# huster-wgm/SRCGAN

Hardware: AMD Instinct MI355X
Metric: paired SR-CycleGAN train images/sec at x4 256->1024 (higher is better)
Workload: dtype bf16; 1 GPU; Sat2Aerx4 paired G+D step (BASELINE configs[1]): 23-block RRDB generator + 3-layer PatchGAN, 3x256x256->3x1024x1024, batch 16/GPU; per_gpu_batch=16, global_batch=16, parallelism=dp1, gradient_exchange=none (1 rank)

## Files before the change

srcgan_amd/csrc/wgrad_dense.hip:

```cpp
#include "common.h"
#include <type_traits>
#include <stdlib.h>

struct WdSeg { int g0, g1; float* grad; float* bias; int Cin; float alpha; };
struct WdP {
    const void* dy; const void* x; float* slab;
    int B, H, W, G, C, dycoff, xcoff;
    long dypix, dyplane, xpix, xplane;
    int g_base;
    int cin_lim[4];
    int nsplit, tiles_x, tiles_y, ntiles, ncit, want_bias;
    unsigned long long* trace;
};
struct WdRedP {
    const float* slab; int nsplit, ncit, COT, g_base, nseg; WdSeg seg[8]; int accumulate;
};

typedef __attribute__((address_space(3))) s16x4 lds_s16x4_;
__device__ __forceinline__ bf16x8 tr_frag2(const char* p0, const char* p1) {
    s16x4 lo = __builtin_amdgcn_ds_read_tr16_b64_v4i16((lds_s16x4_*)(p0));
    s16x4 hi = __builtin_amdgcn_ds_read_tr16_b64_v4i16((lds_s16x4_*)(p1));
    typedef __attribute__((ext_vector_type(8))) short s16x8;
    s16x8 v = {lo[0], lo[1], lo[2], lo[3], hi[0], hi[1], hi[2], hi[3]};
    return __builtin_bit_cast(bf16x8, v);
// ... 58 lines not shown
                if (pix < DPX && oy < p.H && ox < p.W && ch < p.G)
                    src = dyb + (size_t)(oy * p.W + ox) * p.dypix + wd_chan_off<T>(p.dycoff + ch, p.dyplane);
            } else {
                const int pj = pi - MT * DPP, n = pj / XPP, pix = (pj - n * XPP) * PXP + lpx;
                const int iy = pix / IWT, ix = pix - iy * IWT;
                const int gy = oy0 - 1 + iy, gx = ox0 - 1 + ix;
                const int ch = (cit * NT + n) * 32 + part * D::EPP;
                if (pix < XPX && (unsigned)gy < (unsigned)p.H && (unsigned)gx < (unsigned)p.W && ch < p.C)
                    src = xb + (size_t)(gy * p.W + gx) * p.xpix + wd_chan_off<T>(p.xcoff + ch, p.xplane);
            }
            __builtin_amdgcn_global_load_lds((wd_gptr_t)src, (wd_lptr_t)(ls + pi * 1024), 16, 0, 0);
        }
    };

    if (t_begin < t_end) issue(t_begin, 0);
    int stage = 0;
    for (int t = t_begin; t < t_end; ++t, stage ^= 1) {
        __syncthreads();
        if (t + 1 < t_end) issue(t + 1, stage ^ 1);
        const char* my_d = smem + stage * SBYTES + wm * DBYTES;
        const char* my_x = smem + stage * SBYTES + MT * DBYTES + wn * XBYTES;
        if constexpr (std::is_same<T, float>::value) {
#pragma unroll 2
            for (int kk = 0; kk < TH * TW / 2; ++kk) {
                const int pix = 2 * kk + h;
                const int py = pix / TW, px = pix % TW;
                const float a = *(const float*)(my_d + pix * PB + r * 4);
#pragma unroll
                for (int tap = 0; tap < NTAP; ++tap) {
                    const int ky = tap / 3, kx = tap % 3;
                    const float bv = *(const float*)(my_x + ((py + ky) * IWT + px + kx) * PB + r * 4);
                    acc[tap] = __builtin_amdgcn_mfma_f32_32x32x2f32(a, bv, acc[tap], 0, 0, 0);
                }
                if (do_bias) acc[NTAP] = __builtin_amdgcn_mfma_f32_32x32x2f32(a, 1.0f, acc[NTAP], 0, 0, 0);
            }
        } else {
            const int gq = lane >> 4, idx = lane & 15, qq = idx >> 2, pp = idx & 3;
            const int choff = ((gq & 1) * 16 + 4 * pp) * 2;
            const bf16x8 ones = sg_ones16<T>();
#pragma unroll 2
            for (int kk = 0; kk < TH * 2; ++kk) {
                const int py = kk >> 1, xh = (kk & 1) * 16;
                const int px0 = xh + 8 * h + qq;
                const char* ab = my_d + (py * TW + px0) * PB + choff;
                const bf16x8 a = tr_frag2(ab, ab + 4 * PB);
#pragma unroll
                for (int tap = 0; tap < NTAP; ++tap) {
                    const int ky = tap / 3, kx = tap % 3;
                    const char* bb = my_x + ((py + ky) * IWT + px0 + kx) * PB + choff;
                    acc[tap] = sg_mfma16<T>(a, tr_frag2(bb, bb + 4 * PB), acc[tap]);
                }
                if (do_bias) acc[NTAP] = sg_mfma16<T>(a, ones, acc[NTAP]);
            }
        }
    }

    constexpr int COT = 32 * MT, CIT = 32 * NT;
    float* sp = p.slab + ((size_t)split * p.ncit + cit) * (NTAP + 1) * COT * CIT;
#pragma unroll
    for (int tap = 0; tap <= NTAP; ++tap) {
        if (tap == NTAP && !do_bias) continue;
#pragma unroll
        for (int i = 0; i < 16; ++i) {
            const int row = wm * 32 + 8 * (i >> 2) + 4 * h + (i & 3);
            sp[((size_t)tap * COT + row) * CIT + wn * 32 + r] = acc[tap][i];
        }
    }
}

typedef int wd_v4i __attribute__((ext_vector_type(4)));
__device__ __forceinline__ void wd_dma16(const void* base, int voff, int soff, wd_lptr_t lds) {
    const unsigned long long a = (unsigned long long)base;
    wd_v4i rs;
    rs[0] = __builtin_amdgcn_readfirstlane((int)(a & 0xffffffffu));
    rs[1] = __builtin_amdgcn_readfirstlane((int)((a >> 32) & 0xffffu));
    rs[2] = 0x7fffffff;
    rs[3] = 0x00020000;
    const unsigned dst = __builtin_amdgcn_readfirstlane((unsigned)(unsigned long long)lds);
    unsigned keep;
    asm volatile("s_mov_b32 %0, m0\n\ts_mov_b32 m0, %3\n\ts_nop 0\n\tbuffer_load_dwordx4 %1, %2, %4 offen lds\n\ts_mov_b32 m0, %0"
                 : "=&s"(keep) : "v"(voff), "s"(rs), "s"(dst), "s"(soff) : "memory");
}

#ifndef SG_WD_EXP
#define SG_WD_EXP 0
#endif
template <typename T, int MT, int NT, int TH>
__global__ __launch_bounds__(MT * NT * 64) void wgrad_dense_fast_k(const WdP p) {
    using D = DT<T>;
    constexpr int NW = MT * NT, TW = 32, NTAP = 9;
    constexpr int IHT = TH + 2, IWT = TW + 2;
    constexpr int PB = 64, PXP = 16;
    constexpr int DPX = TH * TW, XPX = IHT * IWT;
    constexpr int DPP = (DPX + PXP - 1) / PXP, XPP = (XPX + PXP - 1) / PXP;
    constexpr int DBYTES = DPP * 1024, XBYTES = XPP * 1024;
    constexpr int NPIECE = MT * DPP + NT * XPP, SBYTES = MT * DBYTES + NT * XBYTES;
    constexpr int IPW = (NPIECE + NW - 1) / NW;
    constexpr int OOB = 0x7fffffff;
#ifndef SG_WD_PPK
#define SG_WD_PPK 0
#endif
    constexpr int PPK = SG_WD_PPK ? SG_WD_PPK : 4;
    static_assert(IPW <= 16, "piece classes are packed 4 bits each into two registers");
    extern __shared__ __attribute__((aligned(1024))) char smem[];

    const int tid = threadIdx.x, lane = tid & 63, r = lane & 31, h = lane >> 5;
    const int wave = __builtin_amdgcn_readfirstlane(tid >> 6);
    const int wm = wave / NT, wn = wave % NT;
    int cit, split;
    {
        const int L = blockIdx.x + gridDim.x * blockIdx.y, nwg = gridDim.x * gridDim.y;
        const int xcd = L & 7, j = L >> 3;
        const int full = (nwg >> 3) * 8;
        const int per = nwg >> 3;
        const int pos = L < full ? xcd * per + j : L;
        cit = pos % p.ncit; split = pos / p.ncit;
        if (split >= p.nsplit) return;
    }
    const bool do_bias = wn == 0 && cit == 0 && p.want_bias;
#ifdef SG_WD_NO_SKIP
    const bool useful = true;
#else
    const bool useful = (cit * NT + wn) * 32 < p.cin_lim[wm] || do_bias;
#endif

#ifndef SG_WD_S16
#define SG_WD_S16 1
#endif
    constexpr bool S16 = SG_WD_S16 != 0;
    int voff[IPW]; long soff[IPW];
    unsigned cls[2] = {0u, 0u};
    {
        const int part = lane & 3, lpx = lane >> 2;
#pragma unroll
        for (int it = 0; it < IPW; ++it) {
            const int pi = it * NW + wave;
            int v = OOB; long so = 0;
            if (pi < MT * DPP) {
                const int m = pi / DPP, pix = (pi - m * DPP) * PXP + lpx;
                const int psw = S16 ? part ^ ((((pix % TW) >> 3) & 1) << 1) : part;
                const int ch = p.g_base + m * 32 + psw * D::EPP;
                if (pix < DPX && ch < p.G) v = ((pix / TW) * p.W + pix % TW) * (int)p.dypix + psw * 16;
                so = (long)wd_chan_off<T>(p.dycoff + p.g_base + m * 32, p.dyplane);
            } else if (pi < NPIECE) {
                const int pj = pi - MT * DPP, n = pj / XPP, pix = (pj - n * XPP) * PXP + lpx;
                const int iy = pix / IWT, ix = pix - iy * IWT;
                const int psw = S16 ? part ^ (((ix >> 3) & 1) << 1) : part;
                const int ch = (cit * NT + n) * 32 + psw * D::EPP;
                if (pix < XPX && ch < p.C) v = (iy * p.W + ix) * (int)p.xpix + psw * 16;
                so = (long)wd_chan_off<T>(p.xcoff + (cit * NT + n) * 32, p.xplane);
                cls[it / 8] |= (unsigned)((iy == 0) | ((iy == IHT - 1) << 1) | ((ix == 0) << 2) | ((ix == IWT - 1) << 3)) << (4 * (it % 8));
            }
            voff[it] = v;
            soff[it] = ((long)__builtin_amdgcn_readfirstlane((int)(so >> 32)) << 32) | (unsigned)__builtin_amdgcn_readfirstlane((int)(so & 0xffffffff));
        }
    }

    f32x16 acc[S16 ? 1 : NTAP + 1];
    f32x4 acq[S16 ? NTAP + 1 : 1][2][2];
#pragma unroll
    for (int a = 0; a < (S16 ? 1 : NTAP + 1); ++a)
#pragma unroll
        for (int i = 0; i < 16; ++i) acc[a][i] = 0.f;
#pragma unroll
    for (int a = 0; a < (S16 ? NTAP + 1 : 1); ++a)
#pragma unroll
        for (int i = 0; i < 16; ++i) acq[a][(i >> 3) & 1][(i >> 2) & 1][i & 3] = 0.f;

    const int t_begin = (int)((long)p.ntiles * split / p.nsplit);
    const int t_end = (int)((long)p.ntiles * (split + 1) / p.nsplit);
    int ty = t_begin % p.tiles_y, tx = (t_begin / p.tiles_y) % p.tiles_x, tb = t_begin / (p.tiles_x * p.tiles_y);
    tx = __builtin_amdgcn_readfirstlane(tx); ty = __builtin_amdgcn_readfirstlane(ty); tb = __builtin_amdgcn_readfirstlane(tb);
    const char* dyo = nullptr; const char* xo = nullptr; unsigned clm[2] = {0u, 0u};
    auto origin = [&]() {
        const long px = ((long)tb * p.H + ty * TH) * p.W + tx * TW;
        dyo = (const char*)p.dy + px * p.dypix;
        xo = (const char*)p.x + (px - p.W - 1) * p.xpix;
        const unsigned m = (unsigned)((ty == 0) | ((ty == p.tiles_y - 1) << 1) | ((tx == 0) << 2) | ((tx == p.tiles_x - 1) << 3));
        clm[0] = cls[0] & (m * 0x11111111u); clm[1] = cls[1] & (m * 0x11111111u);
    };
    auto advance = [&]() { if (++ty == p.tiles_y) { ty = 0; if (++tx == p.tiles_x) { tx = 0; ++tb; } } };
    auto piece = [&](int it, int stage) __attribute__((always_inline)) {
        const int pi = it * NW + wave;
        if (IPW * NW != NPIECE && pi >= NPIECE) return;
        int v = ((clm[it / 8] >> (4 * (it % 8))) & 15u) ? OOB : voff[it];
        if (SG_WD_EXP & 8) v = OOB;
        wd_dma16((pi < MT * DPP ? dyo : xo) + soff[it], v, 0, (wd_lptr_t)(smem + stage * SBYTES + pi * 1024));
    };

    if (t_begin < t_end) {
        origin();
#pragma unroll
        for (int it = 0; it < IPW; ++it) piece(it, 0);
    }
    const int gq = lane >> 4, idx = lane & 15, qq = idx >> 2, pp = idx & 3;
    const int choff = ((gq & 1) * 16 + 4 * pp) * 2;
    const bf16x8 ones = sg_ones16<T>();
    int stage = 0;
    for (int t = t_begin; t < t_end; ++t, stage ^= 1) {
#ifdef SG_TRACE
        const unsigned long long t_arr = __builtin_amdgcn_s_memrealtime();
        __builtin_amdgcn_s_waitcnt(0x0f70);
        const unsigned long long t_land = __builtin_amdgcn_s_memrealtime();
#endif
        __builtin_amdgcn_s_waitcnt(0x0f70);
        __syncthreads();
#ifdef SG_TRACE
        if (p.trace && blockIdx.x == 1 && blockIdx.y == 3 && lane == 0 && t - t_begin >= 8 && t - t_begin < 12)
            p.trace[160 + (t - t_begin - 8) * 8 + wave] = t_arr;
        if (p.trace && blockIdx.x == 1 && blockIdx.y == 3 && wave == 0 && lane == 0 && t - t_begin < 40) {
            p.trace[(t - t_begin) * 4 + 0] = t_arr; p.trace[(t - t_begin) * 4 + 1] = t_land; p.trace[(t - t_begin) * 4 + 2] = __builtin_amdgcn_s_memrealtime();
            p.trace[(t - t_begin) * 4 + 3] = __builtin_readcyclecounter();
        }
#endif
        const bool more = t + 1 < t_end;
        if (more) { advance(); origin(); }
        if (!useful) {
            if (more && !(SG_WD_EXP & 1)) {
#pragma unroll
                for (int it = 0; it < IPW; ++it) piece(it, stage ^ 1);
            }
            continue;
        }
        const char* my_d = smem + stage * SBYTES + wm * DBYTES;
        const char* my_x = smem + stage * SBYTES + MT * DBYTES + wn * XBYTES;
#ifndef SG_WD_PD
#define SG_WD_PD 4
#endif
        if constexpr (S16) {
            constexpr int NG = IHT * 3, PDG = 1;
            bf16x8 fa[TH][2], fb[PDG + 1][2];
            const int kq = lane >> 4;
            const int lb = (8 * kq + qq) * PB + (kq & 1) * 32 + 8 * pp;
            const int mk1 = qq + 1 >= 4 ? 32 : 0, mk2 = qq + 2 >= 4 ? 32 : 0;
            auto rd_b = [&](int G) {
                const int i2 = G / 3, kx = G % 3;
                const char* bb = my_x + (i2 * IWT + kx) * PB;
                const int l0 = lb, l1 = lb ^ (kx == 0 ? 0 : kx == 1 ? mk1 : mk2);
                fb[G % (PDG + 1)][0] = tr_frag2(bb + l0, bb + 4 * PB + l1);
                fb[G % (PDG + 1)][1] = tr_frag2(bb + (l0 ^ 32), bb + 4 * PB + (l1 ^ 32));
            };
            auto rd_a = [&](int py) {
                const char* ab = my_d + py * TW * PB;
                fa[py][0] = tr_frag2(ab + lb, ab + 4 * PB + lb);
                fa[py][1] = tr_frag2(ab + (lb ^ 32), ab + 4 * PB + (lb ^ 32));
            };
            rd_a(0); rd_b(0);
#pragma unroll
            for (int G = 0; G < NG; ++G) {
                const int i2 = G / 3, kx = G % 3;
                if (kx == 1 && i2 + 1 < TH) rd_a(i2 + 1);
                if (G + PDG < NG) rd_b(G + PDG);
                if (more) {
#pragma unroll
                    for (int j = 0; j < 2 * PPK; ++j)
                        if (2 * PPK * G + j < IPW) piece(2 * PPK * G + j, stage ^ 1);
                }
                __builtin_amdgcn_sched_barrier(0);
#pragma unroll
                for (int py = 0; py < TH; ++py) {
                    const int ky = i2 - py;
                    if (ky < 0 || ky > 2) continue;
#pragma unroll
                    for (int mb = 0; mb < 2; ++mb)
#pragma unroll
                        for (int nb = 0; nb < 2; ++nb)
                            acq[ky * 3 + kx][mb][nb] = sg_mfma16s<T>(fa[py][mb], fb[G % (PDG + 1)][nb], acq[ky * 3 + kx][mb][nb]);
                }
                if (do_bias && kx == 0 && (i2 == 0 || i2 >= IHT - 2))
#pragma unroll
                    for (int py = (i2 == 0 ? 0 : i2 == IHT - 2 ? 1 : TH / 2); py < (i2 == 0 ? 1 : i2 == IHT - 2 ? TH / 2 : TH); ++py)
#pragma unroll
                        for (int mb = 0; mb < 2; ++mb) acq[NTAP][mb][0] = sg_mfma16s<T>(fa[py][mb], ones, acq[NTAP][mb][0]);
                __builtin_amdgcn_sched_barrier(0);
            }
        } else {
        constexpr int NGRP = IHT * 3 * 2, PD = SG_WD_PD;
        bf16x8 fa[TH][2], fb[PD + 1];
        auto read_b = [&](int G) {
            const int i2 = G / 6, kx = (G % 6) / 2, xh = G % 2;
            const char* bb = my_x + (i2 * IWT + xh * 16 + 8 * h + qq + kx) * PB + choff;
            fb[G % (PD + 1)] = tr_frag2(bb, bb + 4 * PB);
        };
        auto read_a = [&](int py, int xh) {
            const char* ab = my_d + (py * TW + xh * 16 + 8 * h + qq) * PB + choff;
            fa[py][xh] = tr_frag2(ab, ab + 4 * PB);
        };
        read_a(0, 0); read_b(0); read_a(0, 1);
#pragma unroll
        for (int G = 1; G < PD; ++G) read_b(G);
        constexpr int FA_LEAD = 4;
#ifndef SG_WD_PRIO_K
#define SG_WD_PRIO_K 0
#endif
#pragma unroll
        for (int G = 0; G < NGRP; ++G) {
            if (SG_WD_PRIO_K > 0 && wave >= NW / 2) {
                if (G == 0) __builtin_amdgcn_s_setprio(1);
                if (G == SG_WD_PRIO_K) __builtin_amdgcn_s_setprio(0);
            }
            if ((G + FA_LEAD) % 6 < 2 && (G + FA_LEAD) / 6 >= 1 && (G + FA_LEAD) / 6 < TH) read_a((G + FA_LEAD) / 6, (G + FA_LEAD) % 6);
            if (G + PD < NGRP && !(SG_WD_EXP & 4)) read_b(G + PD);
            if (more && !(SG_WD_EXP & 1)) {
#pragma unroll
                for (int j = 0; j < PPK; ++j)
                    if (PPK * G + j < IPW) piece(PPK * G + j, stage ^ 1);
            }
            __builtin_amdgcn_sched_barrier(0);
#ifdef SG_TRACE
            if (G % 5 == 0 && p.trace && blockIdx.x == 1 && blockIdx.y == 3 && lane == 0 && t - t_begin == 10)
                p.trace[192 + wave * 8 + G / 5] = __builtin_amdgcn_s_memrealtime();
#endif
            const int i2 = G / 6, kx = (G % 6) / 2, xh = G % 2;
#pragma unroll
            for (int py = 0; py < TH; ++py) {
                const int ky = i2 - py;
                if (ky < 0 || ky > 2) continue;
                if (!(SG_WD_EXP & 2)) acc[ky * 3 + kx] = sg_mfma16<T>(fa[py][xh], fb[G % (PD + 1)], acc[ky * 3 + kx]);
                else asm volatile("" :: "v"(fa[py][xh]), "v"(fb[G % (PD + 1)]));
            }
            if (do_bias && kx == 0 && (i2 == 0 || i2 >= IHT - 2))
#pragma unroll
                for (int py = (i2 == 0 ? 0 : i2 == IHT - 2 ? 1 : TH / 2); py < (i2 == 0 ? 1 : i2 == IHT - 2 ? TH / 2 : TH); ++py)
                    acc[NTAP] = sg_mfma16<T>(fa[py][xh], ones, acc[NTAP]);
            __builtin_amdgcn_sched_barrier(0);
        }
        }
    }

    constexpr int COT = 32 * MT, CIT = 32 * NT;
    float* sp = p.slab + ((size_t)split * p.ncit + cit) * (NTAP + 1) * COT * CIT;
    const bool blk_needed = (cit * NT + wn) * 32 < p.cin_lim[wm];
#pragma unroll
    for (int tap = 0; tap <= NTAP; ++tap) {
        if (tap == NTAP ? !do_bias : !blk_needed) continue;
        if constexpr (S16) {
#pragma unroll
            for (int mb = 0; mb < 2; ++mb)
#pragma unroll
                for (int nb = 0; nb < 2; ++nb)
#pragma unroll
                    for (int i = 0; i < 4; ++i) {
                        const int row = wm * 32 + mb * 16 + 4 * (lane >> 4) + i;
                        sp[((size_t)tap * COT + row) * CIT + wn * 32 + nb * 16 + (lane & 15)] = acq[tap][mb][tap == NTAP ? 0 : nb][i];
                    }
        } else {
#pragma unroll
            for (int i = 0; i < 16; ++i) {
                const int row = wm * 32 + 8 * (i >> 2) + 4 * h + (i & 3);
                sp[((size_t)tap * COT + row) * CIT + wn * 32 + r] = acc[tap][i];
            }
        }
    }
}

template <int CIT>
__global__ __launch_bounds__(256) void wgrad_dense_reduce_k(const WdRedP p) {
    __shared__ float red[4][64];
    const long per_split = (long)p.ncit * 10 * p.COT * CIT;
    const int el = threadIdx.x & 63, sl = threadIdx.x >> 6;
    const long e = (long)blockIdx.x * 64 + el;
    float s = 0.f;
    bool wanted = false;
    if (e < per_split) {
        long q = e;
        const int col = (int)(q % CIT); q /= CIT;
        const int row = (int)(q % p.COT); q /= p.COT;
        const int tap = (int)(q % 10);
        const int cit = (int)(q / 10);
        const int g = p.g_base + row, ci = cit * CIT + col;
        for (int k = 0; k < p.nseg; ++k) {
            const WdSeg sg = p.seg[k];
            if (g < sg.g0 || g >= sg.g1) continue;
            wanted = tap == 9 ? (sg.bias && cit == 0 && col == 0) : (sg.grad && ci < sg.Cin);
            break;
        }
    }
    if (wanted) {
        float a0 = 0.f, a1 = 0.f, a2 = 0.f, a3 = 0.f;
        int sp = sl;
        for (; sp + 12 < p.nsplit; sp += 16) {
            a0 += p.slab[(size_t)sp * per_split + e];
            a1 += p.slab[(size_t)(sp + 4) * per_split + e];
            a2 += p.slab[(size_t)(sp + 8) * per_split + e];
            a3 += p.slab[(size_t)(sp + 12) * per_split + e];
        }
        for (; sp < p.nsplit; sp += 4) a0 += p.slab[(size_t)sp * per_split + e];
        s = (a0 + a1) + (a2 + a3);
    }
    red[sl][el] = s;
    __syncthreads();
    if (sl != 0 || !wanted) return;
    s = (red[0][el] + red[1][el]) + (red[2][el] + red[3][el]);
    long q = e;
    const int col = (int)(q % CIT); q /= CIT;
    const int row = (int)(q % p.COT); q /= p.COT;
    const int tap = (int)(q % 10);
    const int cit = (int)(q / 10);
    const int g = p.g_base + row, ci = cit * CIT + col;
    for (int k = 0; k < p.nseg; ++k) {
        const WdSeg sg = p.seg[k];
        if (g < sg.g0 || g >= sg.g1) continue;
        const int co = g - sg.g0;
        const float v = s * sg.alpha;
        if (tap == 9) {
            if (sg.bias && cit == 0 && col == 0) sg.bias[co] = p.accumulate ? sg.bias[co] + v : v;
        } else if (sg.grad && ci < sg.Cin) {
            float* gp = sg.grad + ((size_t)co * sg.Cin + ci) * 9 + tap;
            *gp = p.accumulate ? *gp + v : v;
        }
        return;
    }
}

template <typename T, int MT, int NT, int TH>
static int launch_wd(WdP p, hipStream_t st) {
    constexpr int PB = 32 * (int)sizeof(T), PXP = 64 / (PB / 16);
    constexpr size_t SMEM = 2 * 1024 * ((size_t)MT * ((TH * 32 + PXP - 1) / PXP) + (size_t)NT * (((TH + 2) * 34 + PXP - 1) / PXP));
    static_assert(SMEM <= 160 * 1024, "wgrad_dense tile exceeds LDS");
    void (*kern)(const WdP) = wgrad_dense_k<T, MT, NT, TH>;
    bool fast = false;
    if constexpr (!std::is_same<T, float>::value) {
        static const bool no_fast = sg_env("SRCGAN_WD_SLOW") != nullptr;
        const double span_dy = (double)(TH + 2) * p.W * p.dypix, span_x = (double)(TH + 4) * p.W * p.xpix;
        fast = !no_fast && p.H % TH == 0 && p.W % 32 == 0 && span_dy < 2.0e9 && span_x < 2.0e9 &&
               (p.dyplane == 64 || (p.dycoff + p.g_base) % 32 == 0) && (p.xplane == 64 || p.xcoff % 32 == 0);
        constexpr int IPWF = (MT * (TH * 2) + NT * (((TH + 2) * 34 + 15) / 16) + MT * NT - 1) / (MT * NT);
        if constexpr (IPWF <= 10) { if (fast) kern = wgrad_dense_fast_k<T, MT, NT, TH>; }
        else fast = false;
    }
    static bool attr_set[2] = {false, false};
    if (!attr_set[fast]) {
        SG_HIP(hipFuncSetAttribute((const void*)kern, hipFuncAttributeMaxDynamicSharedMemorySize, (int)SMEM));
        attr_set[fast] = true;
    }
    p.tiles_x = cdiv(p.W, 32);
    p.tiles_y = cdiv(p.H, TH);
    p.ntiles = p.B * p.tiles_x * p.tiles_y;
    if (p.nsplit > p.ntiles) p.nsplit = p.ntiles;
    char cls[96];
    snprintf(cls, sizeof(cls), "wgrad_dense<%s,MT%d,NT%d%s>", sizeof(T) == 4 ? "f32" : (__is_same(T, __bf16) ? "bf16" : "f16"), MT, NT, fast ? ",fast" : "");
    const double px = (double)p.B * p.H * p.W;
    const int rows = (p.G - p.g_base) < 32 * MT ? (p.G - p.g_base) : 32 * MT;
    double pairs = 0.0;
    for (int b = 0; b < MT; ++b) {
        const int rb = rows - 32 * b < 32 ? rows - 32 * b : 32;
        if (rb > 0) pairs += (double)rb * (p.cin_lim[b] < p.C ? p.cin_lim[b] : p.C);
    }
    const int tok = sg_prof_start(cls, 2.0 * px * 9 * pairs, px * (rows + p.C) * sizeof(T), st);
#ifdef SG_TRACE
    static unsigned long long* trace = nullptr;
    if (!trace) SG_HIP(hipMalloc(&trace, 64 * 4 * 8));
    SG_HIP(hipMemsetAsync(trace, 0, 64 * 4 * 8, st));
    p.trace = trace;
#endif
    hipLaunchKernelGGL(kern, dim3((unsigned)p.ncit, (unsigned)p.nsplit), dim3(MT * NT * 64), SMEM, st, p);
#ifdef SG_TRACE
    {
        static int dumps = 0;
        if (sg_env("SRCGAN_TRACE") && dumps < 2 && fast) {
            ++dumps;
            unsigned long long h[64 * 4];
            SG_HIP(hipStreamSynchronize(st));
            SG_HIP(hipMemcpy(h, trace, sizeof(h), hipMemcpyDeviceToHost));
            fprintf(stderr, "[trace] %s (10 ns ticks: arrive at barrier, own DMA landed, barrier exit)\n", cls);
            for (int k = 0; k < 4; ++k) {
                fprintf(stderr, "[trace] step %d arrivals by wave (rel. wave 0):", 8 + k);
                for (int w = 0; w < 8; ++w) fprintf(stderr, " %5lld", (long long)(h[160 + k * 8 + w] - h[160 + k * 8]));
                fprintf(stderr, "\n");
            }
            fprintf(stderr, "[trace] step 10: time of groups 0,5,..,35 by wave (rel. wave 0 group 0)\n");
            for (int w = 0; w < 8; ++w) {
                fprintf(stderr, "[trace]   wave %d:", w);
                for (int g = 0; g < 8; ++g) fprintf(stderr, " %5lld", (long long)(h[192 + w * 8 + g] - h[192]));
                fprintf(stderr, "\n");
            }
            for (int k = 0; k < 40 && h[k * 4]; ++k)
                fprintf(stderr, "[trace] %2d arrive %6lld landed %6lld exit %6lld  shader-clock %5.0f MHz\n", k, (long long)(h[k * 4] - h[0]), (long long)(h[k * 4 + 1] - h[0]), (long long)(h[k * 4 + 2] - h[0]),
                        k ? (double)(h[k * 4 + 3] - h[(k - 1) * 4 + 3]) / (double)(h[k * 4 + 2] - h[(k - 1) * 4 + 2]) * 100.0 : 0.0);
        }
    }
#endif
    sg_prof_stop(tok, st);
    SG_LAUNCH_CHECK();
    return p.nsplit;
}

template <typename T>
static int dispatch_wd(const WdP& p, int mt, int nt, hipStream_t st, int& nsplit_used) {
    constexpr bool F = std::is_same<T, float>::value;
    int rc = -1;
    if (nt == 4) {
        if constexpr (!F) {
            switch (mt) {
                case 1: rc = launch_wd<T, 1, 4, 4>(p, st); break;
                case 2: rc = launch_wd<T, 2, 4, 4>(p, st); break;
            }
        }
    } else if (nt == 3) {
        if constexpr (!F) {
            switch (mt) {
                case 1: rc = launch_wd<T, 1, 3, 4>(p, st); break;
                case 2: rc = launch_wd<T, 2, 3, 4>(p, st); break;
            }
        }
    } else
    switch (mt) {
        case 1: rc = launch_wd<T, 1, 2, F ? 2 : 4>(p, st); break;
        case 2: rc = launch_wd<T, 2, 2, F ? 2 : 4>(p, st); break;
        case 3: rc = launch_wd<T, 3, 2, F ? 2 : 4>(p, st); break;
        case 4: rc = launch_wd<T, 4, 2, F ? 2 : 4>(p, st); break;
    }
    if (rc < 0) SG_FAIL("srcgan_wgrad_dense: bad row-tile count %d", mt);
    nsplit_used = rc;
    return 0;
}

static int wd_nt(int mt, int cin_max, int dtype) { return (sg_is16(dtype) && mt <= 2 && cin_max > 64) ? (cin_max <= 96 ? 3 : 4) : 2; }

static int wd_nsplit(int mt, int nt, int ncit, int dtype, int B, int H, int W) {
    const int th = dtype == SRCGAN_F32 ? 2 : 4;
    const int pb = dtype == SRCGAN_F32 ? 128 : 64;
    const long lds = 2 * ((long)mt * th * 32 * pb + (long)nt * (th + 2) * 34 * pb);
    int per_cu = (int)((160 * 1024) / lds); if (per_cu < 1) per_cu = 1;
    if (per_cu * mt * nt > 16) per_cu = 16 / (mt * nt) > 0 ? 16 / (mt * nt) : 1;
    const long ntiles = (long)B * cdiv(H, th) * cdiv(W, 32);
    long cus = 256;
    if (const char* e = sg_env("SRCGAN_WD_CUS")) { const int v = atoi(e); if (v > 0 && v < 256) cus = v; }
    long ns = (cus * per_cu) / ncit;
    if (ns > ntiles) ns = ntiles;
    return (int)(ns < 1 ? 1 : ns);
}

extern "C" size_t srcgan_wgrad_dense_slab_bytes(int G, int C, int dtype, int B, int H, int W) {
    size_t mx = 0;
    for (int g_base = 0; g_base < G; g_base += 128) {
        const int rows = G - g_base < 128 ? G - g_base : 128, mt = cdiv(rows, 32);
        for (int nt = 2; nt <= (sg_is16(dtype) && mt <= 2 ? 4 : 2); ++nt) {
            const int ncit = cdiv(C, 32 * nt);
// ... 66 lines not shown
```

srcgan_amd/ops.py:

```python
from __future__ import annotations

import ctypes as C
from typing import Optional, Tuple

import torch

from . import _native as N

TORCH_DT = {N.F32: torch.float32, N.BF16: torch.bfloat16, N.F16: torch.float16}


def to_nhwc(x: torch.Tensor, cs: Optional[int] = None, dtype=None) -> torch.Tensor:
    N.require_cuda(x, "to_nhwc")
    dt = N.dtype_id(dtype)
    x = x.contiguous().float()
    B, Cc, H, W = x.shape
    cs = cs or Cc
    out = torch.empty(B, H, W, cs, dtype=TORCH_DT[dt], device=x.device)
    N.check(N.lib().srcgan_nchw_f32_to_nhwc(x.data_ptr(), out.data_ptr(), B, Cc, H, W, cs, dt, N.stream_ptr(x.device)), "to_nhwc")
    return out


def to_nchw(x: torch.Tensor, Cc: Optional[int] = None, coff: int = 0) -> torch.Tensor:
    N.require_cuda(x, "to_nchw")
# ... 58 lines not shown
        (B, H, W), xcs = shape, x.shape[-1]
    else:
        B, H, W, xcs = x.shape
    d.x, d.wp, d.y = x.data_ptr(), wp.data_ptr(), y.data_ptr()
    d.bias = bias.data_ptr() if bias is not None else None
    d.dtype = N.dtype_id(x.dtype)
    d.kh, d.kw, d.stride = kh, kw, stride
    d.B, d.H, d.W, d.Cin, d.x_cs, d.x_coff = B, H, W, Cin or (xcs - x_coff), xcs, x_coff
    if OH is None:
        OH = (H + 2 * pad[0] - kh) // stride + 1
        OW = (W + 2 * pad[1] - kw) // stride + 1
    d.OH, d.OW, d.Cout = OH, OW, Cout
    d.YH, d.YW, d.y_cs, d.y_coff = (y.shape[-3], y.shape[-2], y.shape[-1], y_coff)
    d.pad_y, d.pad_x, d.os, d.oa, d.ob = pad[0], pad[1], os, oa, ob
    if r1 is not None:
        d.r1, d.r1_cs, d.r1_coff, d.r1_cend, d.beta1 = r1.data_ptr(), r1.shape[-1], r1_coff, r1_cend, beta1
    if r2 is not None:
        d.r2, d.r2_cs, d.r2_coff, d.r2_cend, d.beta2 = r2.data_ptr(), r2.shape[-1], r2_coff, r2_cend, beta2
    if mz is not None:
        d.mz, d.mz_cs, d.mz_coff, d.mz_c0 = mz.data_ptr(), mz.shape[-1], mz_coff, mz_c0
    if sign_out is not None:
        d.sign_out = sign_out.data_ptr()
    if sign_in is not None:
        d.sign_in = sign_in.data_ptr()
    d.npar, d.wpar_stride = npar, wpar_stride
    d.alpha, d.slope, d.mslope, d.act = alpha, slope, mslope, int(act)
    d.x_plane, d.y_plane, d.r1_plane, d.r2_plane, d.mz_plane = x_plane, y_plane, r1_plane, r2_plane, mz_plane
    N.check(N.lib().srcgan_conv_igemm(C.byref(d), N.stream_ptr(x.device)), "srcgan_conv_igemm")
    return y


def pack_deconv3x3s2(w: torch.Tensor, dtype=None):
    N.require_cuda(w, "pack_deconv3x3s2")
    lib = N.lib()
    dt = N.dtype_id(dtype)
    cin, cout = w.shape[:2]
    w = w.contiguous().float()
    step = lib.srcgan_packed_weight_bytes(cout, cin, 4, dt)
    wp = torch.zeros(4 * step, dtype=torch.uint8, device=w.device)
    for q in range(4):
        a, b = q >> 1, q & 1
        N.check(lib.srcgan_pack_weight(w.data_ptr(), wp.data_ptr() + q * step, cout, cin, a + 1, b + 1, 9, cout * 9, -6, -2,
                                       (2 if a else 1) * 3 + (2 if b else 1), dt, N.stream_ptr(w.device)), "srcgan_pack_weight")
    return wp, step


def deconv3x3s2(x: torch.Tensor, w: torch.Tensor, bias: Optional[torch.Tensor] = None, relu: bool = False, packed=None,
                y: Optional[torch.Tensor] = None) -> torch.Tensor:
    N.require_cuda(x, "deconv3x3s2")
    B, H, W, _ = x.shape
    cout = w.shape[1]
    wp, step = packed if packed is not None else pack_deconv3x3s2(w, x.dtype)
    if y is None:
        y = torch.empty(B, 2 * H, 2 * W, cout, dtype=x.dtype, device=x.device)
    return conv_igemm(x, wp, y, kh=3, kw=3, stride=2, Cout=cout, OH=H, OW=W, pad=(1, 1), bias=bias, act=relu, slope=0.0, os=2,
                      npar=4, wpar_stride=step)


def conv_wgrad(dy: torch.Tensor, x: torch.Tensor, grad: torch.Tensor, *, kh: int, kw: int, stride: int = 1, Cout: int, Cin: int,
               dy_coff: int = 0, x_coff: int = 0, pad: Tuple[int, int] = (0, 0), layout: Tuple[int, int, int, int, int],
               alpha: float = 1.0, nsplit: Optional[int] = None, accumulate: bool = False,
               bias_grad: Optional[torch.Tensor] = None) -> torch.Tensor:
    N.require_cuda(x, "conv_wgrad")
    lib = N.lib()
    d = N.WgradDesc()
    B, OH, OW, dycs = dy.shape
    _, H, W, xcs = x.shape
    ns = nsplit or lib.srcgan_conv_wgrad_nsplit(B, OH, OW, Cout, Cin, stride)
    slab = torch.empty(lib.srcgan_conv_wgrad_slab_bytes(Cout, Cin, kh, kw, ns), dtype=torch.uint8, device=x.device)
    d.dy, d.x, d.slab, d.grad = dy.data_ptr(), x.data_ptr(), slab.data_ptr(), grad.data_ptr()
    d.bias_grad = bias_grad.data_ptr() if bias_grad is not None else None
    d.dtype = N.dtype_id(x.dtype)
    d.kh, d.kw, d.stride = kh, kw, stride
    d.B, d.H, d.W, d.Cin, d.x_cs, d.x_coff = B, H, W, Cin, xcs, x_coff
    d.OH, d.OW, d.Cout, d.dy_cs, d.dy_coff = OH, OW, Cout, dycs, dy_coff
    d.pad_y, d.pad_x, d.nsplit = pad[0], pad[1], ns
    d.sr, d.sk, d.sty, d.stx, d.off = layout
    d.alpha, d.accumulate = alpha, int(accumulate)
    N.check(lib.srcgan_conv_wgrad(C.byref(d), N.stream_ptr(x.device)), "srcgan_conv_wgrad")
    return grad


def wgrad_dense(dy: torch.Tensor, x: torch.Tensor, segs, *, G: Optional[int] = None, Cc: Optional[int] = None,
                dy_plane: int = 0, x_plane: int = 0, shape: Optional[Tuple[int, int, int]] = None) -> None:
    N.require_cuda(x, "wgrad_dense")
    lib = N.lib()
    d = N.WgradDenseDesc()
    if shape is not None:
        (B, H, W), dycs = shape, dy.shape[-1]
    else:
        B, H, W, dycs = dy.shape
    G = G or dycs
    Cc = Cc or x.shape[-1]
    dt = N.dtype_id(x.dtype)
    slab = torch.empty(lib.srcgan_wgrad_dense_slab_bytes(G, Cc, dt, B, H, W), dtype=torch.uint8, device=x.device)
    d.dy, d.x, d.slab, d.dtype = dy.data_ptr(), x.data_ptr(), slab.data_ptr(), dt
    d.B, d.H, d.W, d.G, d.dy_cs, d.dy_coff, d.C, d.x_cs, d.x_coff = B, H, W, G, dycs, 0, Cc, x.shape[-1], 0
    d.dy_plane, d.x_plane = dy_plane, x_plane
    d.nseg = len(segs)
    for i, (g0, g1, grad, bias, cin, alpha) in enumerate(segs):
        d.seg[i].g0, d.seg[i].g1, d.seg[i].Cin, d.seg[i].alpha = g0, g1, cin, alpha
        d.seg[i].grad = grad.data_ptr() if grad is not None else None
        d.seg[i].bias = bias.data_ptr() if bias is not None else None
    N.check(lib.srcgan_wgrad_dense(C.byref(d), N.stream_ptr(x.device)), "srcgan_wgrad_dense")


def col_sum(a: torch.Tensor, Cc: int, coff: int = 0, scale: float = 1.0) -> torch.Tensor:
    N.require_cuda(a, "col_sum")
    lib = N.lib()
    npix = a.numel() // a.shape[-1]
    out = torch.empty(Cc, dtype=torch.float32, device=a.device)
    scr = torch.empty(2 * lib.srcgan_col_reduce_blocks(npix) * Cc, dtype=torch.float32, device=a.device)
    N.check(lib.srcgan_col_reduce(0, a.data_ptr(), a.shape[-1], coff, None, 0, 0, None, None, npix, Cc, scale,
                                  out.data_ptr(), None, scr.data_ptr(), N.dtype_id(a.dtype), N.stream_ptr(a.device)), "srcgan_col_reduce")
    return out


def rgb_to_gray(x: torch.Tensor) -> torch.Tensor:
    N.require_cuda(x, "rgb_to_gray")
    x = x.contiguous().float()
    B, Cc, H, W = x.shape
    if Cc != 3:
        raise ValueError("rgb_to_gray expects 3 channels")
    out = torch.empty(B, 1, H, W, dtype=torch.float32, device=x.device)
    N.check(N.lib().srcgan_rgb_to_gray(x.data_ptr(), out.data_ptr(), B, H, W, N.stream_ptr(x.device)), "srcgan_rgb_to_gray")
    return out


def bilinear_down(x: torch.Tensor, up: int) -> torch.Tensor:
    N.require_cuda(x, "bilinear_down")
    x = x.contiguous().float()
    B, Cc, H, W = x.shape
    out = torch.empty(B, Cc, H // up, W // up, dtype=torch.float32, device=x.device)
    N.check(N.lib().srcgan_bilinear_down(x.data_ptr(), out.data_ptr(), B, Cc, H, W, up, N.stream_ptr(x.device)), "srcgan_bilinear_down")
    return out


def bilinear_up(x: torch.Tensor, up: int) -> torch.Tensor:
    N.require_cuda(x, "bilinear_up")
    x = x.contiguous().float()
    B, Cc, H, W = x.shape
    out = torch.empty(B, Cc, H * up, W * up, dtype=torch.float32, device=x.device)
    N.check(N.lib().srcgan_bilinear_up(x.data_ptr(), out.data_ptr(), B, Cc, H, W, int(up), N.stream_ptr(x.device)), "srcgan_bilinear_up")
    return out


def nearest_resize(x: torch.Tensor, scale_factor: float) -> torch.Tensor:
    N.require_cuda(x, "nearest_resize")
    x = x.contiguous().float()
    B, Cc, H, W = x.shape
    OH, OW = int(H * scale_factor), int(W * scale_factor)
    out = torch.empty(B, Cc, OH, OW, dtype=torch.float32, device=x.device)
    N.check(N.lib().srcgan_nearest_resize(x.data_ptr(), out.data_ptr(), B, Cc, H, W, OH, OW, N.stream_ptr(x.device)), "srcgan_nearest_resize")
    return out


def _check_scale(x: torch.Tensor, s, channels: int, what: str) -> int:
    if isinstance(s, bool) or not isinstance(s, int) or s not in (2, 4):
        raise ValueError(f"{what}: s must be 2 or 4, got {s!r}")
    if x.dim() != 4 or x.shape[1] != channels:
        raise ValueError(f"{what} expects [B,{channels},H,W], got {tuple(x.shape)}")
    return s


def gray_nearest_down(x: torch.Tensor, s: int) -> torch.Tensor:
    s = _check_scale(x, s, 3, "gray_nearest_down")
    B, _, H, W = x.shape
    if H % s or W % s:
        raise ValueError(f"gray_nearest_down: s={s} must divide H and W, got {tuple(x.shape)}")
    N.require_cuda(x, "gray_nearest_down")
    x = x.detach().contiguous().float()
    out = torch.empty(B, 1, H // s, W // s, dtype=torch.float32, device=x.device)
    N.check(N.lib().srcgan_gray_nearest_down(x.data_ptr(), out.data_ptr(), B, H, W, s, N.stream_ptr(x.device)), "srcgan_gray_nearest_down")
    return out


def rep3_nearest_up(x: torch.Tensor, s: int) -> torch.Tensor:
    s = _check_scale(x, s, 1, "rep3_nearest_up")
    B, _, h, w = x.shape
    if h < 1 or w < 1:
        raise ValueError(f"rep3_nearest_up: empty image {tuple(x.shape)}")
# ... 39 lines not shown
```

Before: 119.5 images/s.

## Reuse activation halo rows across vertical tiles in dense wgrad via LDS ring

The fast dense weight-gradient kernel now keeps the activation tile in a 4-slot LDS ring when NT<=3. Consecutive vertical tiles reuse the two halo rows already loaded for the previous tile, so each tile only DMAs its new rows; the full halo is loaded only when a column restarts. The aim is less redundant global-to-LDS traffic per tile. In exchange, LDS slot indexing, border masking and register pressure all get more complex, and the LDS budget changes. The Python wrapper also gains an accumulate flag.

```diff
diff --git a/srcgan_amd/csrc/wgrad_dense.hip b/srcgan_amd/csrc/wgrad_dense.hip
--- a/srcgan_amd/csrc/wgrad_dense.hip
+++ b/srcgan_amd/csrc/wgrad_dense.hip
@@ -164,6 +164,23 @@
                  : "=&s"(keep) : "v"(voff), "s"(rs), "s"(dst), "s"(soff) : "memory");
 }
 
+template <int MT, int NT, int TH>
+struct WdLds {
+    static constexpr bool RING = NT <= 3;
+    static constexpr int HR = RING ? 2 : 0, XROWS = TH + 2 - HR, NSLOT = RING ? 4 : 2;
+    static constexpr int DPP = TH * 32 / 16, XPP = (XROWS * 34 + 15) / 16;
+    static constexpr int HP0 = RING ? (XROWS - HR) * 34 / 16 : XPP;
+    static constexpr int ND = MT * DPP, NPIECE = ND + NT * XPP;
+    static constexpr int IPW = (NPIECE + MT * NT - 1) / (MT * NT);
+    static constexpr int XBLK = XPP * 1024;
+    static constexpr int DSTRIDE = RING ? ND * 1024 : ND * 1024 + NT * XBLK, XSTRIDE = RING ? NT * XBLK : DSTRIDE;
+    static constexpr int XBASE = RING ? 2 * DSTRIDE : ND * 1024;
+    static constexpr int SMEM = RING ? XBASE + NSLOT * XSTRIDE : 2 * DSTRIDE;
+    static constexpr bool FAST = MT * NT >= 6;
+    static_assert(!FAST || IPW <= 10, "larger piece tables would spill beside 160 accumulators");
+    static_assert(SMEM <= 160 * 1024, "wgrad_dense fast tile exceeds LDS");
+};
+
 #ifndef SG_WD_EXP
 #define SG_WD_EXP 0
 #endif
@@ -173,17 +190,20 @@
     constexpr int NW = MT * NT, TW = 32, NTAP = 9;
     constexpr int IHT = TH + 2, IWT = TW + 2;
     constexpr int PB = 64, PXP = 16;
-    constexpr int DPX = TH * TW, XPX = IHT * IWT;
-    constexpr int DPP = (DPX + PXP - 1) / PXP, XPP = (XPX + PXP - 1) / PXP;
-    constexpr int DBYTES = DPP * 1024, XBYTES = XPP * 1024;
-    constexpr int NPIECE = MT * DPP + NT * XPP, SBYTES = MT * DBYTES + NT * XBYTES;
-    constexpr int IPW = (NPIECE + NW - 1) / NW;
+    using L = WdLds<MT, NT, TH>;
+    constexpr bool RING = L::RING;
+    constexpr int HR = L::HR, XROWS = L::XROWS, NSLOT = L::NSLOT, DPP = L::DPP, XPP = L::XPP, HP0 = L::HP0;
+    constexpr int ND = L::ND, NPIECE = L::NPIECE, IPW = L::IPW;
+    constexpr int DPX = TH * TW, XPX = XROWS * IWT, DBYTES = DPP * 1024;
+    constexpr int DSTAGE = L::DSTRIDE, XBLK = L::XBLK, XSLOT = L::XSTRIDE, XBASE = L::XBASE;
+    static_assert(2 * L::SMEM > 160 * 1024, "wd_nsplit counts one workgroup per CU for this kernel");
     constexpr int OOB = 0x7fffffff;
 #ifndef SG_WD_PPK
 #define SG_WD_PPK 0
 #endif
     constexpr int PPK = SG_WD_PPK ? SG_WD_PPK : 4;
-    static_assert(IPW <= 16, "piece classes are packed 4 bits each into two registers");
+    constexpr int IT0 = ND / NW;
+    static_assert(IPW - IT0 <= 8, "the border classes of a wave's activation pieces are packed 4 bits each into one register");
     extern __shared__ __attribute__((aligned(1024))) char smem[];
 
     const int tid = threadIdx.x, lane = tid & 63, r = lane & 31, h = lane >> 5;
@@ -211,27 +231,28 @@
 #endif
     constexpr bool S16 = SG_WD_S16 != 0;
     int voff[IPW]; long soff[IPW];
-    unsigned cls[2] = {0u, 0u};
+    unsigned cls = 0u;
     {
         const int part = lane & 3, lpx = lane >> 2;
 #pragma unroll
         for (int it = 0; it < IPW; ++it) {
             const int pi = it * NW + wave;
             int v = OOB; long so = 0;
-            if (pi < MT * DPP) {
+            if (pi < ND) {
                 const int m = pi / DPP, pix = (pi - m * DPP) * PXP + lpx;
                 const int psw = S16 ? part ^ ((((pix % TW) >> 3) & 1) << 1) : part;
                 const int ch = p.g_base + m * 32 + psw * D::EPP;
                 if (pix < DPX && ch < p.G) v = ((pix / TW) * p.W + pix % TW) * (int)p.dypix + psw * 16;
                 so = (long)wd_chan_off<T>(p.dycoff + p.g_base + m * 32, p.dyplane);
             } else if (pi < NPIECE) {
-                const int pj = pi - MT * DPP, n = pj / XPP, pix = (pj - n * XPP) * PXP + lpx;
+                const int pj = pi - ND, n = pj / XPP, pix = (pj - n * XPP) * PXP + lpx;
                 const int iy = pix / IWT, ix = pix - iy * IWT;
                 const int psw = S16 ? part ^ (((ix >> 3) & 1) << 1) : part;
                 const int ch = (cit * NT + n) * 32 + psw * D::EPP;
                 if (pix < XPX && ch < p.C) v = (iy * p.W + ix) * (int)p.xpix + psw * 16;
                 so = (long)wd_chan_off<T>(p.xcoff + (cit * NT + n) * 32, p.xplane);
-                cls[it / 8] |= (unsigned)((iy == 0) | ((iy == IHT - 1) << 1) | ((ix == 0) << 2) | ((ix == IWT - 1) << 3)) << (4 * (it % 8));
+                const bool top = RING ? iy < XROWS - 1 : iy == 0;
+                if (it >= IT0) cls |= (unsigned)(top | ((iy == XROWS - 1) << 1) | ((ix == 0) << 2) | ((ix == IWT - 1) << 3)) << (4 * (it - IT0));
             }
             voff[it] = v;
             soff[it] = ((long)__builtin_amdgcn_readfirstlane((int)(so >> 32)) << 32) | (unsigned)__builtin_amdgcn_readfirstlane((int)(so & 0xffffffff));
@@ -253,27 +274,43 @@
     const int t_end = (int)((long)p.ntiles * (split + 1) / p.nsplit);
     int ty = t_begin % p.tiles_y, tx = (t_begin / p.tiles_y) % p.tiles_x, tb = t_begin / (p.tiles_x * p.tiles_y);
     tx = __builtin_amdgcn_readfirstlane(tx); ty = __builtin_amdgcn_readfirstlane(ty); tb = __builtin_amdgcn_readfirstlane(tb);
-    const char* dyo = nullptr; const char* xo = nullptr; unsigned clm[2] = {0u, 0u};
+    const char* dyo = nullptr; const char* xo = nullptr; const char* xoh = nullptr;
+    unsigned clm = 0u, clmh = 0u;
+    int cur = NSLOT - 1, nslot = 0, hslot = 0;
+    bool fresh = RING;
     auto origin = [&]() {
         const long px = ((long)tb * p.H + ty * TH) * p.W + tx * TW;
         dyo = (const char*)p.dy + px * p.dypix;
-        xo = (const char*)p.x + (px - p.W - 1) * p.xpix;
-        const unsigned m = (unsigned)((ty == 0) | ((ty == p.tiles_y - 1) << 1) | ((tx == 0) << 2) | ((tx == p.tiles_x - 1) << 3));
-        clm[0] = cls[0] & (m * 0x11111111u); clm[1] = cls[1] & (m * 0x11111111u);
+        xo = (const char*)p.x + (px + (long)(HR - 1) * p.W - 1) * p.xpix;
+        xoh = xo - (long)XROWS * p.W * p.xpix;
+        hslot = (cur + 1) & (NSLOT - 1); nslot = (cur + 1 + (fresh ? 1 : 0)) & (NSLOT - 1);
+        const unsigned mt = ty == 0, mb = (ty == p.tiles_y - 1) << 1, mlr = ((tx == 0) << 2) | ((tx == p.tiles_x - 1) << 3);
+        clm = ((RING ? 0u : mt) | mb | mlr) * 0x11111111u; clmh = (mt | mlr) * 0x11111111u;
     };
     auto advance = [&]() { if (++ty == p.tiles_y) { ty = 0; if (++tx == p.tiles_x) { tx = 0; ++tb; } } };
-    auto piece = [&](int it, int stage) __attribute__((always_inline)) {
-        const int pi = it * NW + wave;
+    int wv = wave;
+    auto piece = [&](int it, int stage, bool head) __attribute__((always_inline)) {
+        const int pi = it * NW + wv;
         if (IPW * NW != NPIECE && pi >= NPIECE) return;
-        int v = ((clm[it / 8] >> (4 * (it % 8))) & 15u) ? OOB : voff[it];
+        if (head && (pi < ND || (pi - ND) % XPP < HP0)) return;
+        int v = voff[it];
+        if (it >= IT0 && (cls & (head ? clmh : clm) & (15u << (4 * (it - IT0))))) v = OOB;
         if (SG_WD_EXP & 8) v = OOB;
-        wd_dma16((pi < MT * DPP ? dyo : xo) + soff[it], v, 0, (wd_lptr_t)(smem + stage * SBYTES + pi * 1024));
+        const char* const o_d = dyo; const char* const o_x = head ? xoh : xo;
+        const int d_d = stage * DSTAGE + pi * 1024, d_x = XBASE + (head ? hslot : RING ? nslot : stage) * XSLOT + (pi - ND) * 1024;
+        wd_dma16((pi < ND ? o_d : o_x) + soff[it], v, 0, (wd_lptr_t)(smem + (pi < ND ? d_d : d_x)));
+    };
+    auto heads = [&](int stage) __attribute__((always_inline)) {
+        if (!RING || !fresh) return;
+#pragma unroll
+        for (int it = IT0; it < IPW; ++it) piece(it, stage, true);
     };
 
     if (t_begin < t_end) {
         origin();
 #pragma unroll
-        for (int it = 0; it < IPW; ++it) piece(it, 0);
+        for (int it = 0; it < IPW; ++it) piece(it, 0, false);
+        heads(0);
     }
     const int gq = lane >> 4, idx = lane & 15, qq = idx >> 2, pp = idx & 3;
     const int choff = ((gq & 1) * 16 + 4 * pp) * 2;
@@ -295,17 +332,23 @@
             p.trace[(t - t_begin) * 4 + 3] = __builtin_readcyclecounter();
         }
 #endif
+        cur = RING ? nslot : stage;
+        asm volatile("" : "+s"(wv));
+        const int xr_prev = ((cur - 1) & (NSLOT - 1)) * XSLOT + (XROWS - HR) * IWT * PB, xr_cur = cur * XSLOT - HR * IWT * PB;
         const bool more = t + 1 < t_end;
-        if (more) { advance(); origin(); }
+        if (more) { advance(); fresh = RING && ty == 0; origin(); }
+        const bool dma = more && !(SG_WD_EXP & 1);
         if (!useful) {
-            if (more && !(SG_WD_EXP & 1)) {
-#pragma unroll
-                for (int it = 0; it < IPW; ++it) piece(it, stage ^ 1);
+            if (dma) {
+#pragma unroll
+                for (int it = 0; it < IPW; ++it) piece(it, stage ^ 1, false);
+                heads(stage ^ 1);
             }
             continue;
         }
-        const char* my_d = smem + stage * SBYTES + wm * DBYTES;
-        const char* my_x = smem + stage * SBYTES + MT * DBYTES + wn * XBYTES;
+        const char* my_d = smem + stage * DSTAGE + wm * DBYTES;
+        const char* my_x = smem + XBASE + wn * XBLK;
+        auto xrow = [&](int i2) { return my_x + (i2 < HR ? xr_prev : xr_cur) + i2 * IWT * PB; };
 #ifndef SG_WD_PD
 #define SG_WD_PD 4
 #endif
@@ -317,8 +360,10 @@
             const int mk1 = qq + 1 >= 4 ? 32 : 0, mk2 = qq + 2 >= 4 ? 32 : 0;
             auto rd_b = [&](int G) {
                 const int i2 = G / 3, kx = G % 3;
-                const char* bb = my_x + (i2 * IWT + kx) * PB;
-                const int l0 = lb, l1 = lb ^ (kx == 0 ? 0 : kx == 1 ? mk1 : mk2);
+                const char* bb = xrow(i2) + kx * PB;
+                int lbg = lb;
+                if constexpr (!RING) asm volatile("" : "+v"(lbg));
+                const int l0 = lbg, l1 = lbg ^ (kx == 0 ? 0 : kx == 1 ? mk1 : mk2);
                 fb[G % (PDG + 1)][0] = tr_frag2(bb + l0, bb + 4 * PB + l1);
                 fb[G % (PDG + 1)][1] = tr_frag2(bb + (l0 ^ 32), bb + 4 * PB + (l1 ^ 32));
             };
@@ -333,10 +378,11 @@
                 const int i2 = G / 3, kx = G % 3;
                 if (kx == 1 && i2 + 1 < TH) rd_a(i2 + 1);
                 if (G + PDG < NG) rd_b(G + PDG);
-                if (more) {
+                if (dma) {
 #pragma unroll
                     for (int j = 0; j < 2 * PPK; ++j)
-                        if (2 * PPK * G + j < IPW) piece(2 * PPK * G + j, stage ^ 1);
+                        if (2 * PPK * G + j < IPW) piece(2 * PPK * G + j, stage ^ 1, false);
+                    if (G == (IPW + 2 * PPK - 1) / (2 * PPK)) heads(stage ^ 1);
                 }
                 __builtin_amdgcn_sched_barrier(0);
 #pragma unroll
@@ -361,7 +407,7 @@
         bf16x8 fa[TH][2], fb[PD + 1];
         auto read_b = [&](int G) {
             const int i2 = G / 6, kx = (G % 6) / 2, xh = G % 2;
-            const char* bb = my_x + (i2 * IWT + xh * 16 + 8 * h + qq + kx) * PB + choff;
+            const char* bb = xrow(i2) + (xh * 16 + 8 * h + qq + kx) * PB + choff;
             fb[G % (PD + 1)] = tr_frag2(bb, bb + 4 * PB);
         };
         auto read_a = [&](int py, int xh) {
@@ -383,10 +429,11 @@
             }
             if ((G + FA_LEAD) % 6 < 2 && (G + FA_LEAD) / 6 >= 1 && (G + FA_LEAD) / 6 < TH) read_a((G + FA_LEAD) / 6, (G + FA_LEAD) % 6);
             if (G + PD < NGRP && !(SG_WD_EXP & 4)) read_b(G + PD);
-            if (more && !(SG_WD_EXP & 1)) {
+            if (dma) {
 #pragma unroll
                 for (int j = 0; j < PPK; ++j)
-                    if (PPK * G + j < IPW) piece(PPK * G + j, stage ^ 1);
+                    if (PPK * G + j < IPW) piece(PPK * G + j, stage ^ 1, false);
+                if (G == (IPW + PPK - 1) / PPK) heads(stage ^ 1);
             }
             __builtin_amdgcn_sched_barrier(0);
 #ifdef SG_TRACE
@@ -412,6 +459,9 @@
 
     constexpr int COT = 32 * MT, CIT = 32 * NT;
     float* sp = p.slab + ((size_t)split * p.ncit + cit) * (NTAP + 1) * COT * CIT;
+    int tid_e = threadIdx.x;
+    asm volatile("" : "+v"(tid_e));
+    const int lane_e = tid_e & 63, r_e = lane_e & 31, h_e = lane_e >> 5;
     const bool blk_needed = (cit * NT + wn) * 32 < p.cin_lim[wm];
 #pragma unroll
     for (int tap = 0; tap <= NTAP; ++tap) {
@@ -423,14 +473,14 @@
                 for (int nb = 0; nb < 2; ++nb)
 #pragma unroll
                     for (int i = 0; i < 4; ++i) {
-                        const int row = wm * 32 + mb * 16 + 4 * (lane >> 4) + i;
-                        sp[((size_t)tap * COT + row) * CIT + wn * 32 + nb * 16 + (lane & 15)] = acq[tap][mb][tap == NTAP ? 0 : nb][i];
+                        const int row = wm * 32 + mb * 16 + 4 * (lane_e >> 4) + i;
+                        sp[((size_t)tap * COT + row) * CIT + wn * 32 + nb * 16 + (lane_e & 15)] = acq[tap][mb][tap == NTAP ? 0 : nb][i];
                     }
         } else {
 #pragma unroll
             for (int i = 0; i < 16; ++i) {
-                const int row = wm * 32 + 8 * (i >> 2) + 4 * h + (i & 3);
-                sp[((size_t)tap * COT + row) * CIT + wn * 32 + r] = acc[tap][i];
+                const int row = wm * 32 + 8 * (i >> 2) + 4 * h_e + (i & 3);
+                sp[((size_t)tap * COT + row) * CIT + wn * 32 + r_e] = acc[tap][i];
             }
         }
     }
@@ -498,22 +548,23 @@
 template <typename T, int MT, int NT, int TH>
 static int launch_wd(WdP p, hipStream_t st) {
     constexpr int PB = 32 * (int)sizeof(T), PXP = 64 / (PB / 16);
-    constexpr size_t SMEM = 2 * 1024 * ((size_t)MT * ((TH * 32 + PXP - 1) / PXP) + (size_t)NT * (((TH + 2) * 34 + PXP - 1) / PXP));
-    static_assert(SMEM <= 160 * 1024, "wgrad_dense tile exceeds LDS");
+    constexpr size_t SMEM_GEN = 2 * 1024 * ((size_t)MT * ((TH * 32 + PXP - 1) / PXP) + (size_t)NT * (((TH + 2) * 34 + PXP - 1) / PXP));
+    static_assert(SMEM_GEN <= 160 * 1024, "wgrad_dense tile exceeds LDS");
     void (*kern)(const WdP) = wgrad_dense_k<T, MT, NT, TH>;
+    size_t smem = SMEM_GEN;
     bool fast = false;
     if constexpr (!std::is_same<T, float>::value) {
         static const bool no_fast = sg_env("SRCGAN_WD_SLOW") != nullptr;
         const double span_dy = (double)(TH + 2) * p.W * p.dypix, span_x = (double)(TH + 4) * p.W * p.xpix;
         fast = !no_fast && p.H % TH == 0 && p.W % 32 == 0 && span_dy < 2.0e9 && span_x < 2.0e9 &&
                (p.dyplane == 64 || (p.dycoff + p.g_base) % 32 == 0) && (p.xplane == 64 || p.xcoff % 32 == 0);
-        constexpr int IPWF = (MT * (TH * 2) + NT * (((TH + 2) * 34 + 15) / 16) + MT * NT - 1) / (MT * NT);
-        if constexpr (IPWF <= 10) { if (fast) kern = wgrad_dense_fast_k<T, MT, NT, TH>; }
+        using L = WdLds<MT, NT, TH>;
+        if constexpr (L::FAST) { if (fast) { kern = wgrad_dense_fast_k<T, MT, NT, TH>; smem = L::SMEM; } }
         else fast = false;
     }
     static bool attr_set[2] = {false, false};
     if (!attr_set[fast]) {
-        SG_HIP(hipFuncSetAttribute((const void*)kern, hipFuncAttributeMaxDynamicSharedMemorySize, (int)SMEM));
+        SG_HIP(hipFuncSetAttribute((const void*)kern, hipFuncAttributeMaxDynamicSharedMemorySize, (int)smem));
         attr_set[fast] = true;
     }
     p.tiles_x = cdiv(p.W, 32);
@@ -536,7 +587,7 @@
     SG_HIP(hipMemsetAsync(trace, 0, 64 * 4 * 8, st));
     p.trace = trace;
 #endif
-    hipLaunchKernelGGL(kern, dim3((unsigned)p.ncit, (unsigned)p.nsplit), dim3(MT * NT * 64), SMEM, st, p);
+    hipLaunchKernelGGL(kern, dim3((unsigned)p.ncit, (unsigned)p.nsplit), dim3(MT * NT * 64), smem, st, p);
 #ifdef SG_TRACE
     {
         static int dumps = 0;
diff --git a/srcgan_amd/ops.py b/srcgan_amd/ops.py
--- a/srcgan_amd/ops.py
+++ b/srcgan_amd/ops.py
@@ -164,7 +164,8 @@
 
 
 def wgrad_dense(dy: torch.Tensor, x: torch.Tensor, segs, *, G: Optional[int] = None, Cc: Optional[int] = None,
-                dy_plane: int = 0, x_plane: int = 0, shape: Optional[Tuple[int, int, int]] = None) -> None:
+                dy_plane: int = 0, x_plane: int = 0, shape: Optional[Tuple[int, int, int]] = None,
+                accumulate: bool = False) -> None:
     N.require_cuda(x, "wgrad_dense")
     lib = N.lib()
     d = N.WgradDenseDesc()
@@ -178,7 +179,7 @@
     slab = torch.empty(lib.srcgan_wgrad_dense_slab_bytes(G, Cc, dt, B, H, W), dtype=torch.uint8, device=x.device)
     d.dy, d.x, d.slab, d.dtype = dy.data_ptr(), x.data_ptr(), slab.data_ptr(), dt
     d.B, d.H, d.W, d.G, d.dy_cs, d.dy_coff, d.C, d.x_cs, d.x_coff = B, H, W, G, dycs, 0, Cc, x.shape[-1], 0
-    d.dy_plane, d.x_plane = dy_plane, x_plane
+    d.dy_plane, d.x_plane, d.accumulate = dy_plane, x_plane, int(accumulate)
     d.nseg = len(segs)
     for i, (g0, g1, grad, bias, cin, alpha) in enumerate(segs):
         d.seg[i].g0, d.seg[i].g1, d.seg[i].Cin, d.seg[i].alpha = g0, g1, cin, alpha
```

New measurement: 119.7 images/s, median of 6. No clear change (+0.2%).
